# mks0601/ExAvatar_RELEASE

Hardware: AMD Instinct MI355X
Metric: train iters/sec (fwd+bwd raster) at 1024x1024 / ~150k Gaussians (higher is better)
Workload: dtype f32

## Files before the change

exavatar_release_amd/csrc/binning.hip:

```cpp
#include <stdlib.h>
#include "common.h"

namespace exa {

constexpr int SCAN_THREADS = 1024;
constexpr int SC_BLOCK_THREADS = 1024;

__device__ __forceinline__ uint32_t wave_incl_scan(uint32_t v) {
    const int lane = threadIdx.x & 63;
#pragma unroll
    for (int d = 1; d < 64; d <<= 1) {
        const uint32_t n = __shfl_up(v, d, 64);
        if (lane >= d) v += n;
    }
    return v;
}

__device__ __forceinline__ uint32_t block_excl_scan(uint32_t v, uint32_t* s_tmp, uint32_t& total) {
    const int tid = threadIdx.x, wave = tid >> 6, lane = tid & 63, nw = blockDim.x >> 6;
    const uint32_t incl = wave_incl_scan(v);
    if (lane == 63) s_tmp[wave] = incl;
    __syncthreads();
    uint32_t base = 0, tot = 0;
    for (int i = 0; i < nw; ++i) {
// ... 236 lines not shown
#define SCATTER_PHASE(i) do { } while (0)
#endif
    {
        const size_t n16 = bin_zero_bytes(capacity) / 16, per = (n16 + gdx - 1) / gdx;
        const size_t lo = (size_t)blockIdx.x * per, hi = lo + per < n16 ? lo + per : n16;
        for (size_t i = lo + threadIdx.x; i < hi; i += SC_BLOCK) owner[i] = make_uint4(0u, 0u, 0u, 0u);
    }
    SCATTER_PHASE(0);
    uint32_t* s_base = s_dyn;
    uint32_t* s_cnt2 = s_dyn + cells;
    const bool publisher = merged && (int)blockIdx.x == chunks;
    if ((int)blockIdx.x >= chunks && !publisher) {
        if (!merged && chunks == 0 && blockIdx.x == 0 && tid == 0 && a.host_hdr)
            report_header(a.host_hdr, w.header->num_rendered, 0u, 0u, a.hdr_tag);
        return;
    }
    constexpr int PER = CHUNK / SC_BLOCK;
    uint4 r3[PER];
    int ids[PER];
    uint32_t depth_bits[PER];
    uint32_t mine = 0;
    auto load_rows = [&] {
#pragma unroll
        for (int it = 0; it < PER; ++it) {
            ids[it] = blockIdx.x * CHUNK + it * SC_BLOCK + tid;
            r3[it] = make_uint4(0, 0, 0, 0);
            depth_bits[it] = 0;
            if (ids[it] < P) {
                r3[it] = reinterpret_cast<const uint4*>(splats + ids[it])[3];
                depth_bits[it] = reinterpret_cast<const uint4*>(splats + ids[it])[2].w;
            }
        }
    };
    uint32_t D, chunk_off;
    if (merged) {
        unsigned long long* s_tot = reinterpret_cast<unsigned long long*>(s_dyn + 2 * cells);
        unsigned long long* s_bef = s_tot + cells;
        const uint32_t ci = tid < chunks ? chunk_inst[tid] : 0u;
        for (int c = tid; c < cells; c += SC_BLOCK) { s_tot[c] = 0ull; s_bef[c] = 0ull; }
        __syncthreads();
        {
            if ((cells & 1) == 0) {
                const int cp = cells >> 1, G2 = SC_BLOCK / cp;
                const int c2 = tid % cp, q = tid / cp;
                if (q < G2) {
                    unsigned long long tot0 = 0ull, tot1 = 0ull, bef0 = 0ull, bef1 = 0ull;
                    const ulonglong2* m = reinterpret_cast<const ulonglong2*>(chunk_cell) + c2;
#pragma unroll 4
                    for (int r = q; r < chunks; r += G2) {
                        const ulonglong2 v = m[(size_t)r * cp];
                        const unsigned long long lowmask = r < (int)blockIdx.x ? 0xffffffffull : 0ull;
                        tot0 += v.x; tot1 += v.y;
                        bef0 += v.x & lowmask; bef1 += v.y & lowmask;
                    }
                    __hip_atomic_fetch_add(&s_tot[2 * c2], tot0, __ATOMIC_RELAXED, __HIP_MEMORY_SCOPE_WORKGROUP);
                    __hip_atomic_fetch_add(&s_tot[2 * c2 + 1], tot1, __ATOMIC_RELAXED, __HIP_MEMORY_SCOPE_WORKGROUP);
                    __hip_atomic_fetch_add(&s_bef[2 * c2], bef0, __ATOMIC_RELAXED, __HIP_MEMORY_SCOPE_WORKGROUP);
                    __hip_atomic_fetch_add(&s_bef[2 * c2 + 1], bef1, __ATOMIC_RELAXED, __HIP_MEMORY_SCOPE_WORKGROUP);
                }
            } else {
            const int G = SC_BLOCK / cells;
            const int c = tid % cells, q = tid / cells;
            if (q < G) {
                unsigned long long tot = 0ull, bef = 0ull;
                const unsigned long long* m = chunk_cell + c;
#pragma unroll 4
                for (int r = q; r < chunks; r += G) {
                    const unsigned long long v = m[(size_t)r * cells];
                    tot += v;
                    bef += r < (int)blockIdx.x ? (v & 0xffffffffull) : 0ull;
                }
                __hip_atomic_fetch_add(&s_tot[c], tot, __ATOMIC_RELAXED, __HIP_MEMORY_SCOPE_WORKGROUP);
                __hip_atomic_fetch_add(&s_bef[c], bef, __ATOMIC_RELAXED, __HIP_MEMORY_SCOPE_WORKGROUP);
            }
            }
        }
        if (!publisher) load_rows();
        __syncthreads();
        SCATTER_PHASE(1);
        const unsigned long long v = tid < cells ? s_tot[tid] : 0ull;
        const unsigned long long packed = ((unsigned long long)(cell_slots((uint32_t)(v >> 32)) * BATCH) << 32) | (uint32_t)v;
        unsigned long long tot_all, x;
        uint32_t inst_total, cx;
        block_excl_scan_pair(packed, ci, s_tmp64, s_tmp, x, tot_all, cx, inst_total);
        if (tid < cells) s_base[tid] = (uint32_t)x + (uint32_t)s_bef[tid];
        D = (uint32_t)(tot_all >> 32);
        if (tid == (int)blockIdx.x) s_bcast[0] = cx;
        if (publisher) {
            if (tid < cells) w.cell_off[tid] = make_uint2((uint32_t)x, (uint32_t)(x >> 32));
            unsigned long long vt;
            block_excl_scan64(tid < chunks ? ((unsigned long long)w.chunk_tiles[tid] << 32) | w.chunk_vis[tid] : 0ull, s_tmp64, vt);
            const uint32_t vis_total = (uint32_t)vt;
            if (tid == 0) {
                w.cell_off[cells] = make_uint2((uint32_t)tot_all, (uint32_t)(tot_all >> 32));
                w.header->num_rendered = D;
                w.header->overflow = (uint64_t)D > capacity ? 1u : 0u;
                w.header->max_tile_list = (uint32_t)tot_all;
                w.header->num_visible = vis_total;
                w.header->num_instances = inst_total;
                w.header->num_tile_instances = (uint32_t)(vt >> 32);
                if (a.host_hdr) report_header(a.host_hdr, D, (uint64_t)D > capacity ? 1u : 0u, vis_total, a.hdr_tag);
            }
            for (int i = tid; i < XCD_REGIONS * ORDER_CLASSES; i += SC_BLOCK) w.cls_cur[i] = 0u;
            if (tid < 4) w.bwd_meta[tid] = 0u;
            __syncthreads();
            write_cell_order(w, cells, [&](int c) { return (uint32_t)(s_tot[c] >> 32); });
            SCATTER_PHASE(5);
            return;
        }
        __syncthreads();
        chunk_off = s_bcast[0];
        SCATTER_PHASE(2);
        if ((uint64_t)D > capacity) return;
        for (int c = tid; c < cells; c += SC_BLOCK) s_cnt2[c] = 0u;
    } else {
        load_rows();
        D = w.header->num_rendered;
        if (a.host_hdr && blockIdx.x == 0 && threadIdx.x == 0)
            report_header(a.host_hdr, D, (uint64_t)D > capacity ? 1u : 0u, w.header->num_visible, a.hdr_tag);
        if ((uint64_t)D > capacity) {
            if (blockIdx.x == 0 && threadIdx.x == 0) w.header->overflow = 1u;
            return;
        }
        chunk_off = w.chunk_off[blockIdx.x];
        for (int c = tid; c < cells; c += SC_BLOCK) {
            s_cnt2[c] = 0u;
            s_base[c] = w.cell_off[c].x + (uint32_t)chunk_cell[(size_t)blockIdx.x * cells + c];
        }
    }
    __syncthreads();

#pragma unroll
    for (int it = 0; it < PER; ++it) mine += r3[it].z;
    uint32_t total;
    uint32_t off = chunk_off + block_excl_scan(mine, s_tmp, total);
    SCATTER_PHASE(3);
#pragma unroll
    for (int it = 0; it < PER; ++it) {
        if (r3[it].z) {
            splats[ids[it]].inst_off = off;
            off += r3[it].z;
            const int sx0 = r3[it].x & 0xffff, sx1 = r3[it].x >> 16, sy0 = r3[it].y & 0xffff, sy1 = r3[it].y >> 16;
            for (int cy = sy0 >> 3; cy <= (sy1 - 1) >> 3; ++cy)
                for (int cx = sx0 >> 3; cx <= (sx1 - 1) >> 3; ++cx) {
                    const int c = cy * gcx + cx;
                    const uint32_t r = __hip_atomic_fetch_add(&s_cnt2[c], 1u, __ATOMIC_RELAXED,
                                                              __HIP_MEMORY_SCOPE_WORKGROUP);
                    bucket[s_base[c] + r] = make_uint4((uint32_t)ids[it], depth_bits[it], r3[it].x, r3[it].y);
                }
        }
    }
    SCATTER_PHASE(4);
}

constexpr int BIN_THREADS = 1024;
struct CellPart { int cell, part; uint32_t e0, e1, lo, hi, slot0; bool overflow, active; int rank, nparts; };
__device__ __forceinline__ bool cell_part_of(const uint4& d, uint32_t need, uint64_t capacity, CellPart& c) {
    if (d.x == NO_PART) return false;
    c.cell = (int)(d.x & 0xfffu); c.rank = (int)((d.x >> 12) & 0xfffu);
    c.part = (int)((d.x >> 24) & 0xfu); c.nparts = (int)(d.x >> 28) + 1;
    c.overflow = (uint64_t)need > capacity;
    c.lo = d.y; c.hi = c.overflow ? d.y : d.z;
    c.e0 = c.e1 = 0u;
    c.slot0 = d.w;
    c.active = d.z > d.y || c.nparts > 1 || c.part > 0;
    return true;
}
template <int PARTS>
__device__ __forceinline__ CellPart cell_part(const uint4& d, uint32_t active, uint32_t need, uint64_t capacity) {
    CellPart c;
    c.cell = (int)d.x;
    c.part = (int)(blockIdx.x % PARTS);
    c.active = blockIdx.x / PARTS < active;
    c.rank = (int)(blockIdx.x / PARTS); c.nparts = PARTS;
    c.overflow = (uint64_t)need > capacity;
    c.e0 = d.y;
    c.e1 = c.overflow ? d.y : d.z;
    c.slot0 = d.w;
    const uint32_t per = (c.e1 - c.e0 + PARTS - 1) / PARTS;
    c.lo = min(c.e1, c.e0 + (uint32_t)c.part * per);
    c.hi = min(c.e1, c.lo + per);
    return c;
}

template <bool FOOTPRINT>
__device__ __forceinline__ unsigned long long entry_mask(const Splat* __restrict__ splats, const uint4& en, int csx0, int csy0) {
    const uint4* rec = reinterpret_cast<const uint4*>(splats + en.x);
    uint4 r0 = make_uint4(0u, 0u, 0u, 0u), r1 = r0;
    if (FOOTPRINT) { r0 = rec[0]; r1 = rec[1]; }
    const int x0 = max((int)(en.z & 0xffff) - csx0, 0), x1 = min((int)(en.z >> 16) - csx0, CELL_SUBS);
    const int y0 = max((int)(en.w & 0xffff) - csy0, 0), y1 = min((int)(en.w >> 16) - csy0, CELL_SUBS);
    const float xl0 = (float)((csx0 + x0) * SUB) - __uint_as_float(r0.x), yl0 = (float)((csy0 + y0) * SUB) - __uint_as_float(r0.y);
    const Footprint fp = make_footprint(__uint_as_float(r1.x), __uint_as_float(r1.y), __uint_as_float(r1.z), __uint_as_float(r1.w),
                                        fmaxf(fabsf(xl0), fabsf(xl0 + (float)((x1 - x0) * SUB))),
                                        fmaxf(fabsf(yl0), fabsf(yl0 + (float)((y1 - y0) * SUB))));
    unsigned long long mask = 0ull;
    for (int y = y0; y < y1; ++y) {
        int c0 = x0, c1 = x1 - 1;
        if (fp.test) {
            float xa, xb;
            const float yl = yl0 + (float)((y - y0) * SUB);
            if (!footprint_band(fp, yl, yl + (float)(SUB - 1), xa, xb)) continue;
            if (xa <= xb) {
                const float m = 1e-3f * (1.0f + fmaxf(fabsf(xa), fabsf(xb)));
                const float lo = clampf((xa - m - (float)(SUB - 1) - xl0) * (1.0f / SUB), -1.0e6f, 1.0e6f);
                const float hi = clampf((xb + m - xl0) * (1.0f / SUB), -1.0e6f, 1.0e6f);
                c0 = max(x0, x0 + (int)ceilf(lo));
                c1 = min(x1 - 1, x0 + (int)floorf(hi));
            }
        }
        if (c1 < c0) continue;
        mask |= (unsigned long long)((2u << c1) - (1u << c0)) << (y * CELL_SUBS);
    }
    return mask;
}

template <bool FOOTPRINT, int PARTS>
__global__ __launch_bounds__(BIN_THREADS) void subtile_count_kernel(Batch<BinArgs> batch) {
    __shared__ uint32_t s_cnt[SUBS_PER_CELL];
    const BinArgs& a = batch.v[blockIdx.y];
    int cells = a.grid.cells;
    const int gcx = a.grid.cx;
    const uint4* __restrict__ part_desc = a.tw.part_desc;
    const ExaRasterHeader* header = a.tw.header;
    uint32_t* __restrict__ part_cnt = a.tw.part_cnt;
    uint4* bucket = a.bw.bucket;
    const Splat* __restrict__ splats = a.splats;
    const uint64_t capacity = a.capacity;
    EXA_TOGETHER(cells, gcx, part_desc, header, part_cnt, bucket, splats, capacity);
    if ((int)blockIdx.x >= cells * PARTS) return;
    uint4 d = uniform_word(part_desc[blockIdx.x]);
    const uint32_t need = uniform_word(header->num_rendered);
    EXA_TOGETHER(d.x, d.y, d.z, d.w, need);
    CellPart cp;
    if (!cell_part_of(d, need, capacity, cp) || !cp.active) return;
    const int tid = threadIdx.x;
    if (tid < SUBS_PER_CELL) s_cnt[tid] = 0u;
    __syncthreads();
    const int csx0 = (cp.cell % gcx) * CELL_SUBS, csy0 = (cp.cell / gcx) * CELL_SUBS;
    for (uint32_t e = cp.lo + tid; e < cp.hi; e += BIN_THREADS) {
        uint4 en = bucket[e];
        asm("" : "+v"(en.x) : "v"(en.y), "v"(en.z), "v"(en.w));
        const unsigned long long mask = entry_mask<FOOTPRINT>(splats, en, csx0, csy0);
        for (unsigned long long m = mask; m; m &= m - 1)
            __hip_atomic_fetch_add(&s_cnt[__builtin_ctzll(m)], 1u, __ATOMIC_RELAXED, __HIP_MEMORY_SCOPE_WORKGROUP);
        reinterpret_cast<uint2*>(bucket + e)[1] = make_uint2((uint32_t)mask, (uint32_t)(mask >> 32));
    }
    __syncthreads();
    if (tid < SUBS_PER_CELL) part_cnt[(size_t)blockIdx.x * SUBS_PER_CELL + tid] = s_cnt[tid];
}

template <int PARTS>
__global__ __launch_bounds__(BIN_THREADS) void subtile_bin_kernel(Batch<BinArgs> batch) {
    __shared__ uint32_t s_off[SUBS_PER_CELL];
    __shared__ uint32_t s_cnt2[SUBS_PER_CELL];
    const BinArgs& a = batch.v[blockIdx.y];
    int cells = a.grid.cells;
    const uint4* part_desc = a.tw.part_desc;
    const ExaRasterHeader* header = a.tw.header;
    const uint32_t* part_cnt = a.tw.part_cnt;
    uint2* ranges = a.tw.ranges;
    uint8_t* cls_code = a.tw.cls_code;
    uint32_t* cell_long = a.tw.cell_long;
    const uint4* bucket = a.bw.bucket;
    uint4* owner = a.bw.owner;
    unsigned long long* keys = a.bw.keys;
    const uint64_t capacity = a.capacity;
    EXA_TOGETHER(cells, part_desc, header, part_cnt, ranges, cls_code, cell_long, bucket, owner, keys, capacity);
    if ((int)blockIdx.x >= cells * PARTS) return;
    uint4 d = uniform_word(part_desc[blockIdx.x]);
    const uint32_t need = uniform_word(header->num_rendered);
    EXA_TOGETHER(d.x, d.y, d.z, d.w, need);
    CellPart cp;
    if (!cell_part_of(d, need, capacity, cp)) return;
    if (!cp.active || cp.overflow) {
        if (cp.part == 0) {
            if (threadIdx.x < SUBS_PER_CELL) {
                ranges[cp.cell * SUBS_PER_CELL + threadIdx.x] = make_uint2(0u, 0u);
                cls_code[cp.cell * SUBS_PER_CELL + threadIdx.x] = (uint8_t)0;
            }
            if (threadIdx.x == 0) cell_long[cp.rank] = 0u;
        }
        return;
    }
    const int cell = cp.cell, tid = threadIdx.x;
    const uint32_t e_first = cp.lo + (uint32_t)tid;
    const uint4 en_first = bucket[min(e_first, max(cp.hi, 1u) - 1u)];
    if (tid < 64) {
        uint32_t n = 0, before = 0;
        const size_t first = (size_t)blockIdx.x - (size_t)cp.part;
#pragma unroll 4
        for (int p = 0; p < cp.nparts; ++p) {
            const uint32_t v = part_cnt[(first + p) * SUBS_PER_CELL + tid];
            before += p < cp.part ? v : 0u;
            n += v;
        }
        const uint32_t nslot = n ? (n + BATCH - 1) / BATCH + 1 : 0u;
        const uint32_t incl = wave_incl_scan(nslot);
        const uint32_t begin = cp.overflow ? 0u : cp.slot0 + (incl - nslot) * BATCH;
        s_off[tid] = begin + before;
        s_cnt2[tid] = 0u;
        if (cp.part == 0) {
            const unsigned long long longer = __ballot(n > (uint32_t)BATCH);
            if (tid == 0) cell_long[cp.rank] = (uint32_t)__popcll(longer);
            ranges[cell * SUBS_PER_CELL + tid] = make_uint2(begin, begin + n);
            cls_code[cell * SUBS_PER_CELL + tid] = (uint8_t)length_class(n);
            for (uint32_t bq = 0; bq + 1 < nslot; ++bq)
                owner[begin / BATCH + bq] = make_uint4((uint32_t)(cell * SUBS_PER_CELL + tid) + 1u, begin, n, 0u);
        }
    }
    __syncthreads();
    auto scatter = [&](const uint4& en) {
        const unsigned long long key = ((unsigned long long)en.y << 32) | en.x;
        for (unsigned long long m = ((unsigned long long)en.w << 32) | en.z; m; m &= m - 1) {
            const int s = __builtin_ctzll(m);
            const uint32_t r = __hip_atomic_fetch_add(&s_cnt2[s], 1u, __ATOMIC_RELAXED, __HIP_MEMORY_SCOPE_WORKGROUP);
            keys[s_off[s] + r] = key;
        }
    };
    if (e_first < cp.hi) scatter(en_first);
    for (uint32_t e = e_first + BIN_THREADS; e < cp.hi; e += BIN_THREADS) scatter(bucket[e]);
}

template <bool FOOTPRINT>
__global__ __launch_bounds__(BIN_THREADS) void subtile_count_bin_kernel(Batch<BinArgs> batch) {
    __shared__ uint32_t s_cnt[SUBS_PER_CELL], s_off[SUBS_PER_CELL], s_cnt2[SUBS_PER_CELL];
    const BinArgs& a = batch.v[blockIdx.y];
    int cells = a.grid.cells;
    const int gcx = a.grid.cx;
    const uint4* cell_desc = a.tw.cell_desc;
    const ExaRasterHeader* header = a.tw.header;
    uint2* ranges = a.tw.ranges;
    uint8_t* cls_code = a.tw.cls_code;
    uint32_t* cell_long = a.tw.cell_long;
    uint4* bucket = a.bw.bucket;
    uint4* owner = a.bw.owner;
    unsigned long long* keys = a.bw.keys;
    const Splat* splats = a.splats;
    const uint64_t capacity = a.capacity;
    EXA_TOGETHER(cells, gcx, cell_desc, header, ranges, cls_code, cell_long, bucket, owner, keys, splats, capacity);
    if ((int)blockIdx.x >= cells) return;
    uint4 d = uniform_word(cell_desc[blockIdx.x]);
    const uint32_t active = uniform_word(header->active_cells), need = uniform_word(header->num_rendered);
    EXA_TOGETHER(d.x, d.y, d.z, d.w, active, need);
    const CellPart cp = cell_part<1>(d, active, need, capacity);
    const int cell = cp.cell, tid = threadIdx.x;
    if (!cp.active) {
        if (tid < SUBS_PER_CELL) {
            ranges[cell * SUBS_PER_CELL + tid] = make_uint2(0u, 0u);
            cls_code[cell * SUBS_PER_CELL + tid] = (uint8_t)0;
        }
        if (tid == 0) cell_long[blockIdx.x] = 0u;
        return;
    }
    if (tid < SUBS_PER_CELL) s_cnt[tid] = 0u;
    __syncthreads();
    const int csx0 = (cell % gcx) * CELL_SUBS, csy0 = (cell / gcx) * CELL_SUBS;
    for (uint32_t e = cp.lo + tid; e < cp.hi; e += BIN_THREADS) {
        uint4 en = bucket[e];
        asm("" : "+v"(en.x) : "v"(en.y), "v"(en.z), "v"(en.w));
        const unsigned long long mask = entry_mask<FOOTPRINT>(splats, en, csx0, csy0);
        for (unsigned long long m = mask; m; m &= m - 1)
            __hip_atomic_fetch_add(&s_cnt[__builtin_ctzll(m)], 1u, __ATOMIC_RELAXED, __HIP_MEMORY_SCOPE_WORKGROUP);
        reinterpret_cast<uint2*>(bucket + e)[1] = make_uint2((uint32_t)mask, (uint32_t)(mask >> 32));
    }
    __syncthreads();
    if (tid < 64) {
        const uint32_t n = s_cnt[tid];
        const uint32_t nslot = n ? (n + BATCH - 1) / BATCH + 1 : 0u;
        const uint32_t incl = wave_incl_scan(nslot);
        const uint32_t begin = cp.overflow ? 0u : cp.slot0 + (incl - nslot) * BATCH;
        s_off[tid] = begin;
        s_cnt2[tid] = 0u;
        const unsigned long long longer = __ballot(n > (uint32_t)BATCH);
        if (tid == 0) cell_long[blockIdx.x] = (uint32_t)__popcll(longer);
        ranges[cell * SUBS_PER_CELL + tid] = make_uint2(begin, begin + n);
        cls_code[cell * SUBS_PER_CELL + tid] = (uint8_t)length_class(n);
        for (uint32_t bq = 0; bq + 1 < nslot; ++bq)
            owner[begin / BATCH + bq] = make_uint4((uint32_t)(cell * SUBS_PER_CELL + tid) + 1u, begin, n, 0u);
    }
    __syncthreads();
    for (uint32_t e = cp.lo + tid; e < cp.hi; e += BIN_THREADS) {
        const uint4 en = bucket[e];
        const unsigned long long key = ((unsigned long long)en.y << 32) | en.x;
        for (unsigned long long m = ((unsigned long long)en.w << 32) | en.z; m; m &= m - 1) {
            const int s = __builtin_ctzll(m);
            const uint32_t r = __hip_atomic_fetch_add(&s_cnt2[s], 1u, __ATOMIC_RELAXED, __HIP_MEMORY_SCOPE_WORKGROUP);
            keys[s_off[s] + r] = key;
        }
    }
}

hipError_t launch_zero(void* p, size_t bytes, hipStream_t s) {
    if (bytes == 0) return hipSuccess;
    const size_t n16 = (bytes + 15) / 16;
    const int blocks = (int)((n16 + BLOCK - 1) / BLOCK < 2048 ? (n16 + BLOCK - 1) / BLOCK : 2048);
    zero_kernel<<<blocks, BLOCK, 0, s>>>(static_cast<uint4*>(p), n16);
    return hipGetLastError();
}

hipError_t launch_cell_scan(const BinArgs* a, int K, hipStream_t s) {
    const Batch<BinArgs> b = make_batch(a, K);
    int cells = 0;
    for (int k = 0; k < K; ++k) cells = max(cells, a[k].grid.cells);
    if (cells > 0) col_scan_kernel<<<dim3((cells + COL_W - 1) / COL_W, K), SCAN_THREADS, 0, s>>>(b);
    cell_scan_kernel<<<dim3(1, K), SCAN_THREADS, 0, s>>>(b);
    return hipGetLastError();
}

hipError_t launch_cell_scatter(const BinArgs* a, int K, hipStream_t s) {
    const Batch<BinArgs> b = make_batch(a, K);
    int chunks = 0, cells = 0;
    for (int k = 0; k < K; ++k) {
        chunks = max(chunks, a[k].chunks);
        cells = max(cells, a[k].grid.cells);
    }
    chunks = a[0].merged ? chunks + 1 : max(chunks, 1);
    cell_scatter_kernel<<<dim3(chunks, K), SC_BLOCK, (size_t)cells * (a[0].merged ? 24 : 8), s>>>(b);
    return hipGetLastError();
}

hipError_t launch_subtile_bin(const BinArgs* a, int K, hipStream_t s) {
    const Batch<BinArgs> b = make_batch(a, K);
    int cells = 0;
    for (int k = 0; k < K; ++k) cells = max(cells, a[k].grid.cells);
    if (cells == 0) return hipSuccess;
    const bool footprint = dev_knobs().footprint;
    const int single_cells = dev_knobs().single_cells;
    if (cells >= single_cells || cells > 1024) {
        if (footprint) subtile_count_bin_kernel<true><<<dim3(cells, K), BIN_THREADS, 0, s>>>(b);
        else subtile_count_bin_kernel<false><<<dim3(cells, K), BIN_THREADS, 0, s>>>(b);
    } else {
        if (footprint) subtile_count_kernel<true, BIN_PARTS><<<dim3(cells * BIN_PARTS, K), BIN_THREADS, 0, s>>>(b);
        else subtile_count_kernel<false, BIN_PARTS><<<dim3(cells * BIN_PARTS, K), BIN_THREADS, 0, s>>>(b);
        subtile_bin_kernel<BIN_PARTS><<<dim3(cells * BIN_PARTS, K), BIN_THREADS, 0, s>>>(b);
    }
    return hipGetLastError();
}

}
```

exavatar_release_amd/csrc/render_fwd.hip:

```cpp
#include <stdlib.h>
#include "blend.h"

namespace exa {

constexpr int RBLOCK = 64;

constexpr int SORT_TILE = 2048;
constexpr int SBLOCK = 256;

template <int E>
__device__ __forceinline__ void lds_merge_sort(const unsigned long long* gkeys, int n, uint32_t* __restrict__ sorted,
                                               unsigned long long* keys_out, unsigned long long* buf, int tid) {
    constexpr int NPAD = SBLOCK * E;
    const int lane = tid & 63;
    unsigned long long key[E];
#pragma unroll
    for (int e = 0; e < E; ++e) {
        const int i = e * SBLOCK + tid;
        key[e] = i < n ? gkeys[i] : ~0ull;
        buf[i] = key[e];
    }
    __syncthreads();
    {
        uint32_t rank[E];
// ... 228 lines not shown
            const uint32_t bkt = (uint32_t)min(NB - 1, (int)f);
            bs[e] = bkt | (__hip_atomic_fetch_add(&cnt[bkt], 1u, __ATOMIC_RELAXED, __HIP_MEMORY_SCOPE_WORKGROUP) << 16);
        }
    }
    wave_lds_fence();
    uint32_t c[E], sum = 0u, mx = 0u;
#pragma unroll
    for (int e = 0; e < E; ++e) { c[e] = cnt[lane * E + e]; sum += c[e]; mx = max(mx, c[e]); }
    uint32_t incl = sum;
#pragma unroll
    for (int d = 1; d < 64; d <<= 1) {
        const uint32_t o = (uint32_t)__shfl_up((int)incl, d, 64);
        if (lane >= d) incl += o;
    }
#pragma unroll
    for (int d = 32; d > 0; d >>= 1) mx = max(mx, (uint32_t)__shfl_xor((int)mx, d, 64));
    if (mx > (uint32_t)BUCKET_MAX) {
        wave_rank_sort_staged<E>(key, n, sorted, keys_out, buf, lane);
        return;
    }
    uint32_t run = incl - sum;
#pragma unroll
    for (int e = 0; e < E; ++e) { cnt[lane * E + e] = run; run += c[e]; }
    wave_lds_fence();
#pragma unroll
    for (int e = 0; e < E; ++e)
        if (e * 64 + lane < n) buf[cnt[bs[e] & 0xffffu] + (bs[e] >> 16)] = key[e];
    wave_lds_fence();
#pragma unroll
    for (int e = 0; e < E; ++e) {
        if (e * 64 + lane < n) {
            const uint32_t bkt = bs[e] & 0xffffu;
            const uint32_t s0 = cnt[bkt], s1 = bkt + 1u < (uint32_t)NB ? cnt[bkt + 1u] : (uint32_t)n;
            uint32_t rank = s0;
            for (uint32_t j = s0; j < s1; ++j) rank += buf[j] < key[e] ? 1u : 0u;
            sorted[rank] = (uint32_t)key[e];
            if (keys_out) keys_out[rank] = key[e];
        }
    }
}

template <int R>
__device__ __forceinline__ void rank_sort_list(const unsigned long long* __restrict__ gkeys, int n, int first,
                                               uint32_t* __restrict__ sorted, unsigned long long* s_keys, int tid) {
    unsigned long long mine[R];
    uint32_t rank[R];
#pragma unroll
    for (int r = 0; r < R; ++r) {
        const int i = first + r * SBLOCK + tid;
        mine[r] = i < n ? gkeys[i] : ~0ull;
        rank[r] = 0;
    }
    for (int tile = 0; tile < n; tile += SORT_TILE) {
        const int tn = min(SORT_TILE, n - tile);
        __syncthreads();
        for (int i = tid; i < ((tn + 1) & ~1); i += SBLOCK) s_keys[i] = i < tn ? gkeys[tile + i] : ~0ull;
        __syncthreads();
        const ulonglong2* s2 = reinterpret_cast<const ulonglong2*>(s_keys);
#pragma unroll 4
        for (int j = 0; j < (tn + 1) / 2; ++j) {
            const ulonglong2 kk = s2[j];
#pragma unroll
            for (int r = 0; r < R; ++r) {
                rank[r] += (kk.x < mine[r]) ? 1u : 0u;
                rank[r] += (kk.y < mine[r]) ? 1u : 0u;
            }
        }
    }
#pragma unroll
    for (int r = 0; r < R; ++r)
        if (first + r * SBLOCK + tid < n) sorted[rank[r]] = (uint32_t)mine[r];
}

constexpr int ORDER_WGS = 32;
constexpr int ORDER_BINS = XCD_REGIONS * ORDER_CLASSES;
constexpr int ORDER_LDS_WORDS = 3 * ORDER_BINS + XCD_REGIONS * (BWD_ORDER_DEPTH + 1);
template <typename RangeOf>
__device__ __forceinline__ void order_slots(const TileWs& w, uint32_t* __restrict__ bwd_order, int subtiles, int part, int tid,
                                            uint32_t* __restrict__ lds, RangeOf range_of) {
    uint32_t* const s_off = lds;
    uint32_t* const s_cnt = lds + ORDER_BINS;
    uint32_t* const s_base = lds + 2 * ORDER_BINS;
    uint32_t* const s_bbase = lds + 3 * ORDER_BINS;
    const int lane = tid & 63;
#ifdef EXA_PROBE_SORTLINE
#define ORDER_STAMP(ph) do { if (tid == 0) w.part_cnt[2 * (subtiles + ORDER_WGS) + part * 8 + (ph)] = (uint32_t)wall_clock64(); } while (0)
#else
#define ORDER_STAMP(ph) do {} while (0)
#endif
    ORDER_STAMP(0);
    for (int i = tid; i < ORDER_BINS; i += SBLOCK) s_cnt[i] = 0u;
    __syncthreads();
    const uint4* __restrict__ codes = reinterpret_cast<const uint4*>(w.cls_code);
    const int n16 = subtiles / 16;
    for (int base = 0; base < n16; base += SBLOCK * 4) {
        uint4 v[4];
#pragma unroll
        for (int i = 0; i < 4; ++i) {
            const int idx = base + i * SBLOCK + tid;
            v[i] = idx < n16 ? codes[idx] : make_uint4(0u, 0u, 0u, 0u);
        }
#pragma unroll
        for (int i = 0; i < 4; ++i) {
            const int idx = base + i * SBLOCK + tid;
            const uint32_t word[4] = {v[i].x, v[i].y, v[i].z, v[i].w};
            if ((word[0] | word[1] | word[2] | word[3]) == 0u) continue;
#pragma unroll
            for (int j = 0; j < 16; ++j) {
                const uint32_t cls = (word[j >> 2] >> (8 * (j & 3))) & 0xffu;
                if (cls) atomicAdd(&s_cnt[xcd_region((idx & 3) * 16 + j) * ORDER_CLASSES + cls], 1u);
            }
        }
    }
    __syncthreads();
    ORDER_STAMP(1);
    {
        constexpr int RPW = (XCD_REGIONS + SBLOCK / 64 - 1) / (SBLOCK / 64);
        const int cls = lane == 63 ? 0 : 63 - lane;
        uint32_t v[RPW], incl[RPW];
#pragma unroll
        for (int j = 0; j < RPW; ++j) {
            const int x = (tid >> 6) + j * (SBLOCK / 64);
            v[j] = incl[j] = x < XCD_REGIONS ? s_cnt[x * ORDER_CLASSES + cls] : 0u;
        }
#pragma unroll
        for (int d = 1; d < 64; d <<= 1) {
#pragma unroll
            for (int j = 0; j < RPW; ++j) {
                const uint32_t o = __shfl_up(incl[j], d, 64);
                if (lane >= d) incl[j] += o;
            }
        }
#pragma unroll
        for (int j = 0; j < RPW; ++j) {
            const int x = (tid >> 6) + j * (SBLOCK / 64);
            if (x < XCD_REGIONS) s_off[x * ORDER_CLASSES + cls] = incl[j] - v[j];
        }
    }
    __syncthreads();
    for (int i = tid; i < ORDER_BINS; i += SBLOCK) s_cnt[i] = 0u;
    if (tid < XCD_REGIONS) {
        uint32_t more[BWD_ORDER_DEPTH];
#pragma unroll
        for (int b = 0; b < BWD_ORDER_DEPTH; ++b) more[b] = s_off[tid * ORDER_CLASSES + 4 * b];
        uint32_t run = 0u;
#pragma unroll
        for (int b = 0; b < BWD_ORDER_DEPTH; ++b) { s_bbase[tid * (BWD_ORDER_DEPTH + 1) + b] = run; run += more[b]; }
        s_bbase[tid * (BWD_ORDER_DEPTH + 1) + BWD_ORDER_DEPTH] = run;
    }
    __syncthreads();
    uint32_t M[XCD_REGIONS];
#pragma unroll
    for (int x = 0; x < XCD_REGIONS; ++x) M[x] = s_bbase[x * (BWD_ORDER_DEPTH + 1) + BWD_ORDER_DEPTH];
    uint32_t m_min = M[0], deep_base = M[0];
#pragma unroll
    for (int x = 1; x < XCD_REGIONS; ++x) { m_min = min(m_min, M[x]); deep_base += M[x]; }
    if (part == 0 && tid == 0) { w.bwd_meta[0] = deep_base; w.bwd_meta[2] = bwd_order ? BWD_ORDER_MAGIC : 0u; }
    ORDER_STAMP(2);
    const int per = (subtiles + ORDER_WGS - 1) / ORDER_WGS;
    const int lo = part * per, hi = min(subtiles, lo + per);
    for (int base = lo; base < hi; base += SBLOCK * 4) {
        uint2 r[4];
        uint32_t rank[4];
#pragma unroll
        for (int i = 0; i < 4; ++i) {
            const int st = base + i * SBLOCK + tid;
            r[i] = st < hi ? range_of(st) : make_uint2(0u, 0u);
        }
#pragma unroll
        for (int i = 0; i < 4; ++i) {
            const int st = base + i * SBLOCK + tid;
            const bool valid = st < hi;
            const int cls = length_class(r[i].y - r[i].x), x = xcd_region(st & 63);
            const bool is_empty = valid && cls == 0;
            unsigned long long mine = 0ull;
#pragma unroll
            for (int xr = 0; xr < XCD_REGIONS; ++xr) {
                const unsigned long long m = __ballot(is_empty && x == xr);
                if (x == xr) mine = m;
            }
            const int leader = is_empty ? __ffsll((long long)mine) - 1 : lane;
            uint32_t b0 = 0u;
            if (cls) b0 = atomicAdd(&s_cnt[x * ORDER_CLASSES + cls], 1u);
            else if (is_empty && lane == leader) b0 = atomicAdd(&s_cnt[x * ORDER_CLASSES], (uint32_t)__popcll(mine));
            b0 = (uint32_t)__shfl((int)b0, leader, 64);
            rank[i] = b0 + (is_empty ? (uint32_t)__popcll(mine & ((1ull << lane) - 1ull)) : 0u);
        }
        ORDER_STAMP(3);
        __syncthreads();
        {
            constexpr int BPT = (ORDER_BINS + SBLOCK - 1) / SBLOCK;
            uint32_t c[BPT], got[BPT];
#pragma unroll
            for (int j = 0; j < BPT; ++j) c[j] = j * SBLOCK + tid < ORDER_BINS ? s_cnt[j * SBLOCK + tid] : 0u;
#pragma unroll
            for (int j = 0; j < BPT; ++j) got[j] = c[j] ? atomicAdd(&w.cls_cur[j * SBLOCK + tid], c[j]) : 0u;
#pragma unroll
            for (int j = 0; j < BPT; ++j)
                if (j * SBLOCK + tid < ORDER_BINS) s_base[j * SBLOCK + tid] = s_off[j * SBLOCK + tid] + got[j];
        }
        __syncthreads();
        ORDER_STAMP(4);
#pragma unroll
        for (int i = 0; i < 4; ++i) {
            const int st = base + i * SBLOCK + tid;
            if (st < hi) {
                const int cls = length_class(r[i].y - r[i].x), x = xcd_region(st & 63);
                const uint32_t k = s_base[x * ORDER_CLASSES + cls] + rank[i];
                w.slots[k * XCD_REGIONS + x] = make_uint4(r[i].x, r[i].y, (uint32_t)st, 0u);
                const uint32_t nb = (r[i].y - r[i].x + BATCH - 1) / BATCH, slot0 = r[i].x / BATCH;
                for (uint32_t b = 0; bwd_order && b < nb; ++b) {
                    uint32_t q;
                    if (b < (uint32_t)BWD_ORDER_DEPTH) {
                        const uint32_t kb = s_bbase[x * (BWD_ORDER_DEPTH + 1) + b] + k;
                        q = kb * XCD_REGIONS + (uint32_t)x;
                        if (kb >= m_min) {
                            q = 0u;
#pragma unroll
                            for (int xo = 0; xo < XCD_REGIONS; ++xo) q += min(M[xo], kb) + (xo < x && M[xo] > kb ? 1u : 0u);
                        }
                    } else {
                        q = deep_base + atomicAdd(&w.bwd_meta[1], 1u);
                    }
                    bwd_order[q] = slot0 + b;
                }
            }
        }
        __syncthreads();
        for (int i = tid; i < ORDER_BINS; i += SBLOCK) s_cnt[i] = 0u;
        __syncthreads();
        ORDER_STAMP(5);
    }
#undef ORDER_STAMP
}

__global__ __launch_bounds__(SBLOCK) void sort_short_kernel(Batch<RenderFwdArgs> batch) {
    __shared__ __attribute__((aligned(16))) unsigned long long s_buf[(SBLOCK / 64) * 64];
    const RenderFwdArgs& a = batch.v[blockIdx.y];
    const int wave = threadIdx.x >> 6, lane = threadIdx.x & 63;
    const int idx = (int)blockIdx.x * (SBLOCK / 64) + wave;
    if (idx >= a.grid.subtiles) return;
    if (idx >= (int)a.tw.header->active_cells * SUBS_PER_CELL) return;
    const int st = (int)a.tw.cell_desc[idx >> 6].x * SUBS_PER_CELL + (idx & 63);
    const uint2 range = a.tw.ranges[st];
    const int n = (int)(range.y - range.x);
    if (n > 0 && n <= 64)
        wave_rank_sort64(a.bw.keys + range.x, n, a.bw.sorted + range.x, a.keep_sorted_keys ? a.bw.keys + range.x : nullptr,
                         s_buf + wave * 64, lane);
}

template <bool KEEP, int MIN_N>
__device__ __forceinline__ void sort_list_workgroup(const RenderFwdArgs& a, int n, unsigned long long* gkeys, uint32_t* sorted,
                                                    unsigned long long* s_buf, uint32_t* s_cnt, uint32_t* s_misc, int tid) {
    unsigned long long* const keys_out = KEEP ? gkeys : nullptr;
    if (n > SORT_TILE) {
        for (int first = 0; first < n; first += 8 * SBLOCK) rank_sort_list<8>(gkeys, n, first, sorted, s_buf, tid);
        if (keys_out) {
            __threadfence_block();
            __syncthreads();
            for (int i = tid; i < n; i += SBLOCK) {
                const uint32_t id = sorted[i];
                keys_out[i] = ((unsigned long long)__float_as_uint(a.splats[id].depth) << 32) | id;
            }
        }
        return;
    }
    bool done;
    if (MIN_N < 256 && n <= 256) done = lds_bucket_sort<1>(gkeys, n, sorted, keys_out, s_buf, s_cnt, s_misc, tid);
    else if (MIN_N < 512 && n <= 512) done = lds_bucket_sort<2>(gkeys, n, sorted, keys_out, s_buf, s_cnt, s_misc, tid);
    else if (n <= 1024) done = lds_bucket_sort<4>(gkeys, n, sorted, keys_out, s_buf, s_cnt, s_misc, tid);
    else done = lds_bucket_sort<8>(gkeys, n, sorted, keys_out, s_buf, s_cnt, s_misc, tid);
    if (done) return;
    __syncthreads();
    if (MIN_N < 256 && n <= 256) lds_merge_sort<1>(gkeys, n, sorted, keys_out, s_buf, tid);
    else if (MIN_N < 512 && n <= 512) lds_merge_sort<2>(gkeys, n, sorted, keys_out, s_buf, tid);
    else if (n <= 1024) lds_merge_sort<4>(gkeys, n, sorted, keys_out, s_buf, tid);
    else lds_merge_sort<8>(gkeys, n, sorted, keys_out, s_buf, tid);
}

template <bool SPLIT, bool KEEP>
__global__ __launch_bounds__(SBLOCK) __attribute__((amdgpu_waves_per_eu(6, 6))) void sort_subtiles_kernel(Batch<RenderFwdArgs> batch) {
    __shared__ __attribute__((aligned(16))) unsigned long long s_buf[SORT_TILE];
    __shared__ uint32_t s_cnt[SORT_TILE];
    __shared__ uint32_t s_misc[16];
    const RenderFwdArgs& a = batch.v[blockIdx.y];
    if ((int)blockIdx.x >= a.grid.subtiles + ORDER_WGS) return;
    const int tid = threadIdx.x;
#ifdef EXA_PROBE_SORTLINE
    struct TL { const RenderFwdArgs& a; unsigned long long t0; int tid;
        __device__ ~TL() { __syncthreads(); if (tid == 0) { a.tw.part_cnt[2 * blockIdx.x] = (uint32_t)t0; a.tw.part_cnt[2 * blockIdx.x + 1] = (uint32_t)wall_clock64(); } } } tl{a, (unsigned long long)wall_clock64(), tid};
#endif
    if (blockIdx.x < ORDER_WGS) {
        static_assert(ORDER_LDS_WORDS <= SORT_TILE, "order_slots borrows the bucket counters of the sort");
        order_slots(a.tw, a.store_ctx ? reinterpret_cast<uint32_t*>(a.bw.bucket) : nullptr, a.grid.subtiles, (int)blockIdx.x, tid,
                    s_cnt, [&](int st) { return a.tw.ranges[st]; });
        return;
    }
#ifdef EXA_PROBE_SORT
    const unsigned long long t0 = __builtin_readcyclecounter();
#endif
    if (blockIdx.x == ORDER_WGS && tid == 0 && (uint64_t)a.tw.header->num_rendered > a.capacity) a.tw.header->overflow = 1u;
    const int wg = (int)blockIdx.x - ORDER_WGS;
    if (wg >= (int)a.tw.header->active_cells * SUBS_PER_CELL) return;
    if (SPLIT && a.tw.cell_long[wg >> 6] == 0u) return;
    const int st = (int)a.tw.cell_desc[wg >> 6].x * SUBS_PER_CELL + (wg & 63);
    const uint2 range = a.tw.ranges[st];
    const int n = (int)(range.y - range.x);
    if (n == 0) return;
    unsigned long long* gkeys = a.bw.keys + range.x;
    uint32_t* sorted = a.bw.sorted + range.x;
    unsigned long long* const keys_out = KEEP ? gkeys : nullptr;
    if (n <= 64) {
        if (!SPLIT && tid < 64) wave_rank_sort64(gkeys, n, sorted, keys_out, s_buf, tid);
        return;
    }
    sort_list_workgroup<KEEP, 64>(a, n, gkeys, sorted, s_buf, s_cnt, s_misc, tid);
#ifdef EXA_PROBE_SORT
    __syncthreads();
    if (tid == 0) a.tw.part_cnt[st] = (uint32_t)(__builtin_readcyclecounter() - t0);
#endif
}

template <bool KEEP>
__global__ __launch_bounds__(SBLOCK) __attribute__((amdgpu_waves_per_eu(6, 6))) void sort_subtiles_quads_kernel(Batch<RenderFwdArgs> batch,
                                                                                                                int quads) {
    constexpr int WK = WAVE_KEYS > 0 ? WAVE_KEYS : 256;
    constexpr int TAIL_STRIDE = WK / BATCH + 1;
    static_assert(4 * WK * 12 <= SORT_TILE * 12, "four wave regions share the buffers of the workgroup sort");
    __shared__ __attribute__((aligned(16))) unsigned long long s_buf[SORT_TILE + SORT_TILE / 2];
    __shared__ uint32_t s_misc[16];
    uint32_t* const s_cnt = reinterpret_cast<uint32_t*>(s_buf + SORT_TILE);
    const RenderFwdArgs& a = batch.v[blockIdx.y];
    const int tid = threadIdx.x;
#ifdef EXA_PROBE_SORTLINE
    struct TL { const RenderFwdArgs& a; unsigned long long t0; int tid;
        __device__ ~TL() { __syncthreads(); if (tid == 0) { a.tw.part_cnt[2 * blockIdx.x] = (uint32_t)t0; a.tw.part_cnt[2 * blockIdx.x + 1] = (uint32_t)wall_clock64(); } } } tl{a, (unsigned long long)wall_clock64(), tid};
#endif
    if (blockIdx.x < ORDER_WGS) {
        static_assert(ORDER_LDS_WORDS <= SORT_TILE, "order_slots borrows the bucket counters of the sort");
        order_slots(a.tw, a.store_ctx ? reinterpret_cast<uint32_t*>(a.bw.bucket) : nullptr, a.grid.subtiles, (int)blockIdx.x, tid,
                    s_cnt, [&](int st) { return a.tw.ranges[st]; });
        return;
    }
    const int q = (int)blockIdx.x - ORDER_WGS;
    if (q < quads) {
        if (q == 0 && tid == 0 && (uint64_t)a.tw.header->num_rendered > a.capacity) a.tw.header->overflow = 1u;
        if (q * 4 >= a.grid.subtiles || q * 4 >= (int)a.tw.header->active_cells * SUBS_PER_CELL) return;
        const int wave = __builtin_amdgcn_readfirstlane(tid >> 6), lane = tid & 63;
        const int idx = q * 4 + wave;
        const int st = (int)a.tw.cell_desc[idx >> 6].x * SUBS_PER_CELL + (idx & 63);
        const uint2 range = a.tw.ranges[st];
        const int n = (int)(range.y - range.x);
        if (n > 0 && n <= WK) {
            unsigned long long* gkeys = a.bw.keys + range.x;
            uint32_t* sorted = a.bw.sorted + range.x;
            unsigned long long* const keys_out = KEEP ? gkeys : nullptr;
            unsigned long long* const w_buf = s_buf + wave * (WK * 12 / 8);
            uint32_t* const w_cnt = reinterpret_cast<uint32_t*>(w_buf + WK);
            if (n <= 64) wave_rank_sort64(gkeys, n, sorted, keys_out, w_buf, lane);
            else if (n <= 128) wave_bucket_sort<2>(gkeys, n, sorted, keys_out, w_buf, w_cnt, lane);
            else if (WK == 256 || n <= 256) wave_bucket_sort<4>(gkeys, n, sorted, keys_out, w_buf, w_cnt, lane);
            else wave_bucket_sort<WK / 64>(gkeys, n, sorted, keys_out, w_buf, w_cnt, lane);
        }
        return;
    }
    const uint32_t slot = (uint32_t)(q - quads) * (uint32_t)TAIL_STRIDE;
    if ((uint64_t)slot * BATCH >= a.capacity) return;
    const uint4 own = a.bw.owner[slot];
    const int n = (int)own.z;
    if (own.x == 0u || n <= WK || slot - own.y / BATCH >= (uint32_t)TAIL_STRIDE) return;
    sort_list_workgroup<KEEP, WK>(a, n, a.bw.keys + own.y, a.bw.sorted + own.y, s_buf, s_cnt, s_misc, tid);
}

template <bool STORE, bool TWO>
__global__ __launch_bounds__(RBLOCK) void render_fwd_kernel(Batch<RenderFwdArgs> batch) {
    __shared__ BatchLds s_b;

    const RenderFwdArgs& a = batch.v[blockIdx.y];
    int subtiles = a.grid.subtiles;
    const int gW = a.grid.W, gH = a.grid.H, gcx = a.grid.cx;
    const uint4* __restrict__ slots = a.tw.slots;
    const Splat* __restrict__ splats = a.splats;
    const uint32_t* __restrict__ sorted_all = a.bw.sorted;
    float* ckpt_all = a.bw.ckpt;
    unsigned long long* bmask = a.bw.bmask;
    uint2* fwd_exit = a.tw.fwd_exit;
    const float* __restrict__ bg = a.bg;
    float* out_color = a.out_color; float* out_depth = a.out_depth; float* out_alpha = a.out_alpha;
    const uint2* ranges = a.tw.ranges;
    const Splat* __restrict__ splats2 = a.splats2;
    const float* src_color = a.src_color; const float* src_depth = a.src_depth; const float* src_alpha = a.src_alpha;
    const float* src_bg = a.src_bg;
    if (TWO)
        EXA_TOGETHER(subtiles, gW, gH, gcx, slots, splats, sorted_all, ckpt_all, bmask, fwd_exit, bg, out_color, out_depth, out_alpha,
                     ranges, splats2, src_color, src_depth, src_alpha, src_bg);
    else
        EXA_TOGETHER(subtiles, gW, gH, gcx, slots, splats, sorted_all, ckpt_all, bmask, fwd_exit, bg, out_color, out_depth, out_alpha);
    if ((int)blockIdx.x >= subtiles) return;
    const int lane = threadIdx.x;
#ifdef EXA_PROBE_FWD
    const unsigned long long t0 = wall_clock64();
#endif
    uint4 slot = uniform_word(slots[blockIdx.x]);
    const float bg0 = uniform_word(bg[0]), bg1 = uniform_word(bg[1]), bg2 = uniform_word(bg[2]);
    EXA_TOGETHER(slot.z, slot.x, slot.y, slot.w, bg0, bg1, bg2);
    Grid grid;
    grid.W = gW; grid.H = gH; grid.cx = gcx;
    const SubTile sub = decode_subtile((int)slot.z, grid);
    const int st = sub.st;
    if (sub.ox >= gW || sub.oy >= gH) return;
    const int pxi = sub.ox + (lane & 7), pyi = sub.oy + (lane >> 3);
    const bool inside = pxi < gW && pyi < gH;
    const float fx = (float)pxi, fy = (float)pyi;
    const uint2 range = TWO ? ranges[slot.z] : make_uint2(slot.x, slot.y);
    const int n = (int)(range.y - range.x);
    if (TWO && n == 0 && reuse_a_pixels(src_color, src_bg, bg0, bg1, bg2)) {
        if (inside) {
            const size_t HW = (size_t)gW * gH, pix = (size_t)pyi * gW + pxi;
            const float c0 = src_color[pix], c1 = src_color[HW + pix], c2 = src_color[2 * HW + pix];
            const float d = src_depth[pix], al = src_alpha[pix];
            out_color[pix] = c0; out_color[HW + pix] = c1; out_color[2 * HW + pix] = c2;
            out_depth[pix] = d; out_alpha[pix] = al;
        }
        if (STORE && lane == 0) fwd_exit[st] = make_uint2(0u, 0u);
        return;
    }

    float T = inside ? 1.0f : 0.0f, Tdead = 1.0f;
    v2f Crg = {0.f, 0.f}, Cbd = {0.f, 0.f};
    const uint32_t* __restrict__ sorted = sorted_all + range.x;
    auto record = [&](uint32_t id) -> const float4* {
        if (TWO) return reinterpret_cast<const float4*>(((id & SRC_B) ? splats2 : splats) + (id & ~SRC_B));
        return reinterpret_cast<const float4*>(splats + id);
    };

    uint32_t id_next = 0;
    float2 r0 = make_float2(0.f, 0.f);
    float4 r1 = make_float4(0.f, 0.f, 0.f, 0.f), r2 = r1;
    if (n > 0) {
        const uint32_t id0 = lane < n ? sorted[lane] : 0u;
        if (64 + lane < n) id_next = sorted[64 + lane];
        if (lane < n) {
            const float4* rec = record(id0);
            r0 = *reinterpret_cast<const float2*>(rec); r1 = rec[1]; r2 = rec[2];
        }
    }
    float* ckpt = ckpt_all + (size_t)(range.x / BATCH) * (5 * 64) + lane;
    int entered = 0;
    for (int base = 0; base < n; base += 64) {
        if (__all(T == 0.0f)) break;
        if (STORE && base > 0) {
            float* c = ckpt + (size_t)entered * (5 * 64);
            c[0] = T > 0.0f ? T : -Tdead; c[64] = Crg.x; c[128] = Crg.y; c[192] = Cbd.x; c[256] = Cbd.y;
        }
        ++entered;
        const unsigned long long unsafe = __builtin_amdgcn_ballot_w64(!conic_safe(r1.x, r1.y, r1.z));
        stage_splat(s_b, lane, r0, r1, r2);
        {
            const int jn = base + 64 + lane;
            r0 = make_float2(0.f, 0.f); r1 = make_float4(0.f, 0.f, 0.f, 0.f); r2 = r1;
            if (jn < n) {
                const float4* rec = record(id_next);
                r0 = *reinterpret_cast<const float2*>(rec); r1 = rec[1]; r2 = rec[2];
            }
            if (jn + 64 < n) id_next = sorted[jn + 64];
        }
        wave_lds_fence();
        const int cnt = min(64, n - base);
        unsigned long long blended = 0ull;
        auto blend4 = [&](const Alpha4& e, const float4& c0, const float4& c1, const float4& c2, const float4& c3, int k) -> bool {
#ifdef EXA_FWD_SKIP_VOTE
            const float amax = fmaxf(fmaxf(e.alpha[0], e.alpha[1]), fmaxf(e.alpha[2], e.alpha[3])) * T;
            if (!__any(amax > 0.0f)) return false;
#endif
            const unsigned long long live_mask = __builtin_amdgcn_ballot_w64(T > 0.0f);
            if (STORE) {
                auto vote_bit = [&](int j, uint32_t bit) -> uint32_t {
                    const unsigned long long m = e.took[j] & live_mask;
                    uint32_t r;
                    asm("s_cmp_lg_u64 %1, 0\n\ts_cselect_b32 %0, %2, 0" : "=s"(r) : "s"(m), "s"(bit) : "scc");
                    return r;
                };
                const uint32_t nib = vote_bit(0, 1u) | vote_bit(1, 2u) | vote_bit(2, 4u) | vote_bit(3, 8u);
                blended |= (unsigned long long)nib << k;
            }
            float Tb[4], w[4];
            blend_group4(T, Tdead, live_mask, e.alpha, Tb, w);
            Crg = __builtin_elementwise_fma(v2f{c0.x, c0.y}, v2f{w[0], w[0]}, Crg);
            Cbd = __builtin_elementwise_fma(v2f{c0.z, c0.w}, v2f{w[0], w[0]}, Cbd);
            Crg = __builtin_elementwise_fma(v2f{c1.x, c1.y}, v2f{w[1], w[1]}, Crg);
            Cbd = __builtin_elementwise_fma(v2f{c1.z, c1.w}, v2f{w[1], w[1]}, Cbd);
            Crg = __builtin_elementwise_fma(v2f{c2.x, c2.y}, v2f{w[2], w[2]}, Crg);
            Cbd = __builtin_elementwise_fma(v2f{c2.z, c2.w}, v2f{w[2], w[2]}, Cbd);
            Crg = __builtin_elementwise_fma(v2f{c3.x, c3.y}, v2f{w[3], w[3]}, Crg);
            Cbd = __builtin_elementwise_fma(v2f{c3.z, c3.w}, v2f{w[3], w[3]}, Cbd);
#ifdef EXA_FWD_EXIT4
            return __all(T == 0.0f);
#else
            return (k & 4) ? __all(T == 0.0f) : false;
#endif
        };
        auto group4 = [&](const Ops4& ops, int k) -> bool {
            const float4 c0 = s_b.col[k], c1 = s_b.col[k + 1], c2 = s_b.col[k + 2], c3 = s_b.col[k + 3];
            Alpha4 e = splat_alpha4(ops, fx, fy, true);
            if ((unsafe >> k) & 0xfull) power_guard4(e, ops, (uint32_t)((unsafe >> k) & 0xfull));
            return blend4(e, c0, c1, c2, c3, k);
        };
        Ops4 opsA = load_ops4(s_b, 0);
        for (int k = 0; k < cnt; k += 8) {
            const Ops4 opsB = load_ops4(s_b, (k + 4) & 63);
            if (group4(opsA, k)) break;
            if (k + 4 >= cnt) break;
            opsA = load_ops4(s_b, (k + 8) & 63);
            if (group4(opsB, k + 4)) break;
        }
        if (STORE && lane == 0) bmask[range.x / BATCH + (uint32_t)(entered - 1)] = blended;
        wave_lds_fence();
    }

    const size_t HW = (size_t)gW * gH;
    if (inside) {
        const size_t pix = (size_t)pyi * gW + pxi;
        const float Tf = T > 0.0f ? T : Tdead;
        out_color[pix] = Crg.x + Tf * bg0;
        out_color[HW + pix] = Crg.y + Tf * bg1;
        out_color[2 * HW + pix] = Cbd.x + Tf * bg2;
        out_depth[pix] = Cbd.y;
        out_alpha[pix] = 1.0f - Tf;
    }
    if (STORE) {
        if (lane == 0) fwd_exit[st] = make_uint2((uint32_t)n, (uint32_t)entered);
#ifdef EXA_PROBE_FWD
        if (lane == 0) {
            a.tw.part_cnt[4 * blockIdx.x] = (uint32_t)t0;
            a.tw.part_cnt[4 * blockIdx.x + 1] = (uint32_t)wall_clock64();
            const uint32_t hw = __builtin_amdgcn_s_getreg((31 << 11) | 4), xcc = __builtin_amdgcn_s_getreg((31 << 11) | 20);
            a.tw.part_cnt[4 * blockIdx.x + 2] = (hw & 0xffffu) | ((xcc & 0xfu) << 16);
        }
#endif
        if (n > 0) {
            float* c = ckpt + (size_t)((n + BATCH - 1) / BATCH) * (5 * 64);
            c[0] = T > 0.0f ? T : Tdead; c[64] = Crg.x; c[128] = Crg.y; c[192] = Cbd.x; c[256] = Cbd.y;
        }
    }
}

static int max_subtiles(const RenderFwdArgs* a, int K) {
    int n = 0;
    for (int k = 0; k < K; ++k) n = max(n, a[k].grid.subtiles);
    return n;
}

hipError_t launch_sort_subtiles(const RenderFwdArgs* a, int K, hipStream_t s) {
    const int subtiles = max_subtiles(a, K);
    if (subtiles == 0) return hipSuccess;
    const int split_at = dev_knobs().split_subtiles;
    bool keep = false;
    for (int k = 0; k < K; ++k) keep = keep || a[k].keep_sorted_keys != 0;
    const dim3 grid(subtiles + ORDER_WGS, K);
    if (subtiles >= split_at) {
        sort_short_kernel<<<dim3((subtiles + SBLOCK / 64 - 1) / (SBLOCK / 64), K), SBLOCK, 0, s>>>(make_batch(a, K));
        if (keep) sort_subtiles_kernel<true, true><<<grid, SBLOCK, 0, s>>>(make_batch(a, K));
        else sort_subtiles_kernel<true, false><<<grid, SBLOCK, 0, s>>>(make_batch(a, K));
    } else if (WAVE_KEYS > 0) {
        const int quads = (subtiles + SBLOCK / 64 - 1) / (SBLOCK / 64);
        int tail = 0;
        for (int k = 0; k < K; ++k)
            tail = max(tail, (int)((a[k].capacity / BATCH + WAVE_KEYS / BATCH) / (uint64_t)(WAVE_KEYS / BATCH + 1)));
        const dim3 qgrid(ORDER_WGS + quads + tail, K);
        if (keep) sort_subtiles_quads_kernel<true><<<qgrid, SBLOCK, 0, s>>>(make_batch(a, K), quads);
        else sort_subtiles_quads_kernel<false><<<qgrid, SBLOCK, 0, s>>>(make_batch(a, K), quads);
    } else {
        if (keep) sort_subtiles_kernel<false, true><<<grid, SBLOCK, 0, s>>>(make_batch(a, K));
        else sort_subtiles_kernel<false, false><<<grid, SBLOCK, 0, s>>>(make_batch(a, K));
    }
    return hipGetLastError();
}

#ifndef EXA_FWD_LDS_PAD
#define EXA_FWD_LDS_PAD 0
#endif
hipError_t launch_render_fwd(const RenderFwdArgs* a, int K, hipStream_t s) {
    const int subtiles = max_subtiles(a, K);
    if (subtiles == 0) return hipSuccess;
    constexpr int pad = EXA_FWD_LDS_PAD;
    if (a[0].splats2) {
        if (a[0].store_ctx) render_fwd_kernel<true, true><<<dim3(subtiles, K), RBLOCK, (size_t)pad, s>>>(make_batch(a, K));
        else render_fwd_kernel<false, true><<<dim3(subtiles, K), RBLOCK, (size_t)pad, s>>>(make_batch(a, K));
    } else if (a[0].store_ctx)
        render_fwd_kernel<true, false><<<dim3(subtiles, K), RBLOCK, (size_t)pad, s>>>(make_batch(a, K));
    else
        render_fwd_kernel<false, false><<<dim3(subtiles, K), RBLOCK, (size_t)pad, s>>>(make_batch(a, K));
    return hipGetLastError();
}

}
```

Before: 7996.

## Schedule long-list sort workgroups first via per-cell tail counts

Binning now packs a second count into cell_long: the number of sub-tiles per cell whose list exceeds WAVE_KEYS, stored in the upper 16 bits. The quads sort kernel no longer walks the owner slot array to find long lists. Each tail workgroup prefix-scans these per-cell counts to locate the t-th long list directly, and a front section of tail workgroups is placed before the quad workgroups so that long sorts start early rather than at the end of the grid. This is meant to cut the long-pole tail and the empty tail workgroups, at the cost of a block scan per tail workgroup and a cap on cell count for this path.

Result: no change. 8015 (median of 4 runs) (+0.2%).

```diff
diff --git a/exavatar_release_amd/csrc/binning.hip b/exavatar_release_amd/csrc/binning.hip
--- a/exavatar_release_amd/csrc/binning.hip
+++ b/exavatar_release_amd/csrc/binning.hip
@@ -562,7 +562,8 @@
         s_cnt2[tid] = 0u;
         if (cp.part == 0) {
             const unsigned long long longer = __ballot(n > (uint32_t)BATCH);
-            if (tid == 0) cell_long[cp.rank] = (uint32_t)__popcll(longer);
+            const unsigned long long tails = __ballot(n > (uint32_t)WAVE_KEYS);
+            if (tid == 0) cell_long[cp.rank] = (uint32_t)__popcll(longer) | (uint32_t)__popcll(tails) << 16;
             ranges[cell * SUBS_PER_CELL + tid] = make_uint2(begin, begin + n);
             cls_code[cell * SUBS_PER_CELL + tid] = (uint8_t)length_class(n);
             for (uint32_t bq = 0; bq + 1 < nslot; ++bq)
@@ -633,7 +634,8 @@
         s_off[tid] = begin;
         s_cnt2[tid] = 0u;
         const unsigned long long longer = __ballot(n > (uint32_t)BATCH);
-        if (tid == 0) cell_long[blockIdx.x] = (uint32_t)__popcll(longer);
+        const unsigned long long tails = __ballot(n > (uint32_t)WAVE_KEYS);
+        if (tid == 0) cell_long[blockIdx.x] = (uint32_t)__popcll(longer) | (uint32_t)__popcll(tails) << 16;
         ranges[cell * SUBS_PER_CELL + tid] = make_uint2(begin, begin + n);
         cls_code[cell * SUBS_PER_CELL + tid] = (uint8_t)length_class(n);
         for (uint32_t bq = 0; bq + 1 < nslot; ++bq)
diff --git a/exavatar_release_amd/csrc/render_fwd.hip b/exavatar_release_amd/csrc/render_fwd.hip
--- a/exavatar_release_amd/csrc/render_fwd.hip
+++ b/exavatar_release_amd/csrc/render_fwd.hip
@@ -554,7 +554,7 @@
     if (blockIdx.x == ORDER_WGS && tid == 0 && (uint64_t)a.tw.header->num_rendered > a.capacity) a.tw.header->overflow = 1u;
     const int wg = (int)blockIdx.x - ORDER_WGS;
     if (wg >= (int)a.tw.header->active_cells * SUBS_PER_CELL) return;
-    if (SPLIT && a.tw.cell_long[wg >> 6] == 0u) return;
+    if (SPLIT && (a.tw.cell_long[wg >> 6] & 0xffffu) == 0u) return;
     const int st = (int)a.tw.cell_desc[wg >> 6].x * SUBS_PER_CELL + (wg & 63);
     const uint2 range = a.tw.ranges[st];
     const int n = (int)(range.y - range.x);
@@ -573,11 +573,65 @@
 #endif
 }
 
+
+template <int WK>
+__device__ __forceinline__ uint2 find_long_list(const uint32_t* __restrict__ cell_long, const uint4* __restrict__ cell_desc,
+                                                const uint2* __restrict__ ranges, int cells, uint32_t t, uint32_t* s_lds, int tid) {
+    const int lane = tid & 63, wave = tid >> 6, r0 = tid * 4;
+    uint32_t c[4] = {0u, 0u, 0u, 0u}, cell[4] = {0u, 0u, 0u, 0u};
+    if (r0 < cells) {
+        const uint4 w = reinterpret_cast<const uint4*>(cell_long)[tid];
+#pragma unroll
+        for (int j = 0; j < 4; ++j) cell[j] = cell_desc[min(r0 + j, cells - 1)].x;
+        const uint32_t ww[4] = {w.x, w.y, w.z, w.w};
+#pragma unroll
+        for (int j = 0; j < 4; ++j) c[j] = r0 + j < cells ? ww[j] >> 16 : 0u;
+    }
+    const uint32_t sum = c[0] + c[1] + c[2] + c[3];
+    uint32_t incl = sum;
+#pragma unroll
+    for (int d = 1; d < 64; d <<= 1) {
+        const uint32_t o = (uint32_t)__shfl_up((int)incl, d, 64);
+        if (lane >= d) incl += o;
+    }
+    if (lane == 63) s_lds[wave] = incl;
+    __syncthreads();
+    uint32_t excl = incl - sum, total = 0u;
+#pragma unroll
+    for (int w2 = 0; w2 < SBLOCK / 64; ++w2) {
+        const uint32_t v = s_lds[w2];
+        excl += w2 < wave ? v : 0u;
+        total += v;
+    }
+    if (t >= total) return make_uint2(0u, 0u);
+    if (t >= excl && t - excl < sum) {
+        uint32_t k = t - excl, mine = cell[0];
+#pragma unroll
+        for (int j = 0; j < 3; ++j)
+            if (k >= c[j]) { k -= c[j]; mine = cell[j + 1]; } else break;
+        s_lds[4] = mine; s_lds[5] = k;
+    }
+    __syncthreads();
+    const uint32_t the_cell = s_lds[4], k = s_lds[5];
+    const uint2 r = ranges[the_cell * SUBS_PER_CELL + lane];
+    const unsigned long long longs = __ballot(r.y - r.x > (uint32_t)WK);
+    const bool me = ((longs >> lane) & 1ull) && (uint32_t)__popcll(longs & ((1ull << lane) - 1ull)) == k;
+    const int sel = __ffsll((long long)__ballot(me)) - 1;
+    if (sel < 0) return make_uint2(0u, 0u);
+    return make_uint2(uniform_word((uint32_t)__shfl((int)r.x, sel, 64)), uniform_word((uint32_t)__shfl((int)r.y, sel, 64)));
+}
+
+#ifndef EXA_FRONT_TAIL_SHIFT
+#define EXA_FRONT_TAIL_SHIFT (EXA_WAVE_KEYS == 256 ? 3 : 5)
+#endif
+static_assert(EXA_FRONT_TAIL_SHIFT >= 1, "the front section takes at most half of the sub-tiles");
+static int front_tail_workgroups(int subtiles) { return subtiles >> EXA_FRONT_TAIL_SHIFT; }
+constexpr int QUADS_MAX_CELLS = SBLOCK * 4;
+
 template <bool KEEP>
 __global__ __launch_bounds__(SBLOCK) __attribute__((amdgpu_waves_per_eu(6, 6))) void sort_subtiles_quads_kernel(Batch<RenderFwdArgs> batch,
-                                                                                                                int quads) {
+                                                                                                                int quads, int front) {
     constexpr int WK = WAVE_KEYS > 0 ? WAVE_KEYS : 256;
-    constexpr int TAIL_STRIDE = WK / BATCH + 1;
     static_assert(4 * WK * 12 <= SORT_TILE * 12, "four wave regions share the buffers of the workgroup sort");
     __shared__ __attribute__((aligned(16))) unsigned long long s_buf[SORT_TILE + SORT_TILE / 2];
     __shared__ uint32_t s_misc[16];
@@ -594,8 +648,8 @@
                     s_cnt, [&](int st) { return a.tw.ranges[st]; });
         return;
     }
-    const int q = (int)blockIdx.x - ORDER_WGS;
-    if (q < quads) {
+    const int g = (int)blockIdx.x - ORDER_WGS, q = g - front;
+    if (q >= 0 && q < quads) {
         if (q == 0 && tid == 0 && (uint64_t)a.tw.header->num_rendered > a.capacity) a.tw.header->overflow = 1u;
         if (q * 4 >= a.grid.subtiles || q * 4 >= (int)a.tw.header->active_cells * SUBS_PER_CELL) return;
         const int wave = __builtin_amdgcn_readfirstlane(tid >> 6), lane = tid & 63;
@@ -616,12 +670,11 @@
         }
         return;
     }
-    const uint32_t slot = (uint32_t)(q - quads) * (uint32_t)TAIL_STRIDE;
-    if ((uint64_t)slot * BATCH >= a.capacity) return;
-    const uint4 own = a.bw.owner[slot];
-    const int n = (int)own.z;
-    if (own.x == 0u || n <= WK || slot - own.y / BATCH >= (uint32_t)TAIL_STRIDE) return;
-    sort_list_workgroup<KEEP, WK>(a, n, a.bw.keys + own.y, a.bw.sorted + own.y, s_buf, s_cnt, s_misc, tid);
+    const uint32_t t = (uint32_t)(g < front ? g : g - quads);
+    const uint2 range = find_long_list<WK>(a.tw.cell_long, a.tw.cell_desc, a.tw.ranges, a.grid.cells, t, s_misc + 8, tid);
+    const int n = (int)(range.y - range.x);
+    if (n <= WK) return;
+    sort_list_workgroup<KEEP, WK>(a, n, a.bw.keys + range.x, a.bw.sorted + range.x, s_buf, s_cnt, s_misc, tid);
 }
 
 template <bool STORE, bool TWO>
@@ -814,14 +867,15 @@
         sort_short_kernel<<<dim3((subtiles + SBLOCK / 64 - 1) / (SBLOCK / 64), K), SBLOCK, 0, s>>>(make_batch(a, K));
         if (keep) sort_subtiles_kernel<true, true><<<grid, SBLOCK, 0, s>>>(make_batch(a, K));
         else sort_subtiles_kernel<true, false><<<grid, SBLOCK, 0, s>>>(make_batch(a, K));
-    } else if (WAVE_KEYS > 0) {
+    } else if (WAVE_KEYS > 0 && subtiles <= QUADS_MAX_CELLS * SUBS_PER_CELL) {
         const int quads = (subtiles + SBLOCK / 64 - 1) / (SBLOCK / 64);
         int tail = 0;
         for (int k = 0; k < K; ++k)
             tail = max(tail, (int)((a[k].capacity / BATCH + WAVE_KEYS / BATCH) / (uint64_t)(WAVE_KEYS / BATCH + 1)));
+        const int front = min(tail, front_tail_workgroups(subtiles));
         const dim3 qgrid(ORDER_WGS + quads + tail, K);
-        if (keep) sort_subtiles_quads_kernel<true><<<qgrid, SBLOCK, 0, s>>>(make_batch(a, K), quads);
-        else sort_subtiles_quads_kernel<false><<<qgrid, SBLOCK, 0, s>>>(make_batch(a, K), quads);
+        if (keep) sort_subtiles_quads_kernel<true><<<qgrid, SBLOCK, 0, s>>>(make_batch(a, K), quads, front);
+        else sort_subtiles_quads_kernel<false><<<qgrid, SBLOCK, 0, s>>>(make_batch(a, K), quads, front);
     } else {
         if (keep) sort_subtiles_kernel<false, true><<<grid, SBLOCK, 0, s>>>(make_batch(a, K));
         else sort_subtiles_kernel<false, false><<<grid, SBLOCK, 0, s>>>(make_batch(a, K));
```
